# NVlabs/latentfusion

Measured on AMD Instinct MI355X. Metric: pose-optim iters/sec (reconstruct+render+backward), 16 views, 128^3 voxels, higher is better.
Workload: dtype f32

## Files before the change

### latentfusion_amd/csrc/resample.hip

```cpp
#include "resample_map.h"

namespace {

typedef unsigned u32x4_t __attribute__((ext_vector_type(4)));

struct Tap {
  int x0, y0, z0, x1, y1, z1;
  float tx, ty, tz;
  float mx, my, mz;
};

__device__ __forceinline__ float lattice01(int i, int size, float step) {
  return (i < size / 2) ? step * (float)i : 1.f - step * (float)(size - 1 - i);
}


template <int KIND>
__device__ __forceinline__ void eval_grid(const float* __restrict__ cf, int x, int y, int z,
                                          int W, int H, int D, Steps st, float& gx, float& gy, float& gz,
                                          float& a, float& b, float& k) {
  a = lattice01(x, W, st.w);
  b = lattice01(y, H, st.h);
  k = lattice01(z, D, st.d);
  if (KIND == LF_MAP_O2C) {
    const float ak = a * k, bk = b * k;
    gx = cf[0] + cf[3] * a + cf[6] * b + cf[9] * k + cf[12] * ak + cf[15] * bk;
    gy = cf[1] + cf[4] * a + cf[7] * b + cf[10] * k + cf[13] * ak + cf[16] * bk;
    gz = cf[2] + cf[5] * a + cf[8] * b + cf[11] * k + cf[14] * ak + cf[17] * bk;
  } else {
    const float lx = 2.f * a - 1.f, ly = 2.f * b - 1.f, lz = 2.f * k - 1.f;
    const float n0 = cf[0] * lx + cf[1] * ly + cf[2] * lz + cf[3];
    const float n1 = cf[4] * lx + cf[5] * ly + cf[6] * lz + cf[7];
    const float n2 = cf[8] * lx + cf[9] * ly + cf[10] * lz + cf[11];
    const float dn = cf[12] * lx + cf[13] * ly + cf[14] * lz + cf[15];
    gx = n0 / dn;
    gy = n1 / dn;
    gz = n2;
  }
}

__device__ __forceinline__ void unnormalize_clip(float g, int size, float& pos, float& mult) {
  float p = ((g + 1.f) * (float)size - 1.f) * 0.5f;
  const float hi = (float)(size - 1);
  mult = (p > 0.f && p < hi) ? 0.5f * (float)size : 0.f;
  p = fminf(fmaxf(p, 0.f), hi);
  pos = p;
}

__device__ __forceinline__ Tap make_tap(float gx, float gy, float gz, int W, int H, int D) {
  Tap t;
  float px, py, pz;
  unnormalize_clip(gx, W, px, t.mx);
  unnormalize_clip(gy, H, py, t.my);
  unnormalize_clip(gz, D, pz, t.mz);
  if (!(px == px)) px = 0.f;
  if (!(py == py)) py = 0.f;
  if (!(pz == pz)) pz = 0.f;
  const float fx = floorf(px), fy = floorf(py), fz = floorf(pz);
  t.tx = px - fx; t.ty = py - fy; t.tz = pz - fz;
  t.x0 = (int)fx; t.y0 = (int)fy; t.z0 = (int)fz;
  t.x1 = min(t.x0 + 1, W - 1); t.y1 = min(t.y0 + 1, H - 1); t.z1 = min(t.z0 + 1, D - 1);
  return t;
}

__device__ __forceinline__ unsigned xcd_contiguous(unsigned b, unsigned nb) {
  return (nb % 8 == 0) ? (b % 8) * (nb / 8) + b / 8 : b;
}

static int bwd_vox_per_block(long nvox, int N) {
  long v = nvox * N / 2048;
  int p = 64;
  while (p < 4096 && p * 2 <= v) p <<= 1;
  return p;
}
struct BwdTile { int lx, ly, lz, ntx, nty, ntz; };
static BwdTile bwd_tile(int vpb, int D, int H, int W) {
  int lg = 0;
  while ((1 << lg) < vpb) ++lg;
  BwdTile t;
  t.lx = (lg + 2) / 3; t.ly = (lg + 1) / 3; t.lz = lg / 3;
  t.ntx = (W + (1 << t.lx) - 1) >> t.lx; t.nty = (H + (1 << t.ly) - 1) >> t.ly; t.ntz = (D + (1 << t.lz) - 1) >> t.lz;
  return t;
}

__global__ void __launch_bounds__(256) resample_bwd_coef_reduce(const float* __restrict__ partial,
                                                                int nblk, float* __restrict__ gcoef) {
  const int n = blockIdx.x;
  __shared__ double red[256];
  const int comp = threadIdx.x % 18;
  const int grp = threadIdx.x / 18;
  double s = 0.0;
  if (grp < 14)
    for (int b = grp; b < nblk; b += 14) s += (double)partial[((long)n * nblk + b) * 18 + comp];
  red[threadIdx.x] = (grp < 14) ? s : 0.0;
  __syncthreads();
  if (threadIdx.x < 18) {
    double tot = 0.0;
    for (int g = 0; g < 14; ++g) tot += red[g * 18 + threadIdx.x];
    gcoef[(long)n * 18 + threadIdx.x] = (float)tot;
  }
}

template <int KIND>
__global__ void __launch_bounds__(256) resample_bwd_vol_kernel(
    const float* __restrict__ gout, const float* __restrict__ coef, float* __restrict__ gvol,
    long gvol_bstride, int N, int D, int H, int W, int C, Steps st) {
  const long per_sample = (long)D * H * W * C;
  const int n = blockIdx.y;
  const float* cf = coef + (long)n * LF_MAP_COEFS;
  for (long idx = (long)blockIdx.x * blockDim.x + threadIdx.x; idx < per_sample;
       idx += (long)gridDim.x * blockDim.x) {
    const int c = (int)(idx % C);
    long v = idx / C;
    const int x = (int)(v % W); v /= W;
    const int y = (int)(v % H);
    const int z = (int)(v / H);
    float gx, gy, gz, a, b, k;
    eval_grid<KIND>(cf, x, y, z, W, H, D, st, gx, gy, gz, a, b, k);
    const Tap t = make_tap(gx, gy, gz, W, H, D);
    const float go = gout[(long)n * per_sample + idx];
    float* base = gvol + (long)n * gvol_bstride + c;
    const long sW = C, sH = (long)W * C, sD = (long)H * W * C;
    const float wx1 = t.tx, wx0 = 1.f - t.tx, wy1 = t.ty, wy0 = 1.f - t.ty, wz1 = t.tz, wz0 = 1.f - t.tz;
    atomicAdd(base + t.z0 * sD + t.y0 * sH + t.x0 * sW, go * (wx0 * wy0 * wz0));
    atomicAdd(base + t.z0 * sD + t.y0 * sH + t.x1 * sW, go * (wx1 * wy0 * wz0));
    atomicAdd(base + t.z0 * sD + t.y1 * sH + t.x0 * sW, go * (wx0 * wy1 * wz0));
    atomicAdd(base + t.z0 * sD + t.y1 * sH + t.x1 * sW, go * (wx1 * wy1 * wz0));
    atomicAdd(base + t.z1 * sD + t.y0 * sH + t.x0 * sW, go * (wx0 * wy0 * wz1));
    atomicAdd(base + t.z1 * sD + t.y0 * sH + t.x1 * sW, go * (wx1 * wy0 * wz1));
    atomicAdd(base + t.z1 * sD + t.y1 * sH + t.x0 * sW, go * (wx0 * wy1 * wz1));
    atomicAdd(base + t.z1 * sD + t.y1 * sH + t.x1 * sW, go * (wx1 * wy1 * wz1));
  }
}

typedef unsigned u32;

struct Tap32 {
  u32 o000, o001, o010, o011, o100, o101, o110, o111;
  float tx, ty, tz, mx, my, mz;
};

__device__ __forceinline__ void axis_tap(float g, int size, u32 stride, u32& o0, u32& d1, float& t, float& m) {
  float p;
  unnormalize_clip(g, size, p, m);
  if (!(p == p)) p = 0.f;
  const float f = floorf(p);
  t = p - f;
  const int i0 = (int)f;
  o0 = (u32)i0 * stride;
  d1 = (i0 + 1 <= size - 1) ? stride : 0u;
}

__device__ __forceinline__ Tap32 make_tap32(float gx, float gy, float gz, int W, int H, int D, u32 rec_bytes) {
  Tap32 t;
  u32 x0, dx, y0, dy, z0, dz;
  axis_tap(gx, W, rec_bytes, x0, dx, t.tx, t.mx);
  axis_tap(gy, H, rec_bytes * (u32)W, y0, dy, t.ty, t.my);
  axis_tap(gz, D, rec_bytes * (u32)W * (u32)H, z0, dz, t.tz, t.mz);
  const u32 b00 = z0 + y0, b01 = b00 + dy, b10 = b00 + dz, b11 = b01 + dz;
  t.o000 = b00 + x0; t.o001 = t.o000 + dx;
  t.o010 = b01 + x0; t.o011 = t.o010 + dx;
  t.o100 = b10 + x0; t.o101 = t.o100 + dx;
  t.o110 = b11 + x0; t.o111 = t.o110 + dx;
  return t;
}

__device__ __forceinline__ f32x4 ldrec(__amdgpu_buffer_rsrc_t rs, u32 off) {
  return __builtin_bit_cast(f32x4, __builtin_amdgcn_raw_buffer_load_b128(rs, (int)off, 0, 0));
}

typedef unsigned u32x2_t __attribute__((ext_vector_type(2)));
template <bool B16>
__device__ __forceinline__ f32x4 ldrec_t(__amdgpu_buffer_rsrc_t rs, u32 off) {
  if constexpr (B16)
    return __builtin_convertvector(__builtin_bit_cast(bf16x4r, __builtin_amdgcn_raw_buffer_load_b64(rs, (int)off, 0, 0)), f32x4);
  else
    return __builtin_bit_cast(f32x4, __builtin_amdgcn_raw_buffer_load_b128(rs, (int)off, 0, 0));
}

__device__ __forceinline__ float quad_sum4(float v) {
  const float a = v + __int_as_float(__builtin_amdgcn_update_dpp(0, __float_as_int(v), 0xB1, 0xF, 0xF, true));
  return a + __int_as_float(__builtin_amdgcn_update_dpp(0, __float_as_int(a), 0x4E, 0xF, 0xF, true));
}

__device__ __forceinline__ long vol_offset(int n, long vol_bstride, const int* __restrict__ vol_idx, int vol_n) {
  const int v = vol_idx[n];
  return (long)(v < 0 ? 0 : (v >= vol_n ? vol_n - 1 : v)) * vol_bstride;
}

#define GATHER_KERNEL(stem) stem##_kernel
// ... 78 lines not shown
#endif

int g_bwd_coef_variant = 10;
int g_resample_variant = 3;

}

struct FwdPlan {
  bool vec;
  int lpt, tlx, tly, tlz, nbz;
  dim3 grid;
  Steps st;
};
static int fwd_plan(const float* vol, const float* out, int N, int D, int H, int W, int C, FwdPlan& p) {
  if ((long)D * H * W >= 0x7fffffffL) return LF_EINVAL;
  p.vec = (C % 4 == 0) && lf_aligned16(vol) && lf_aligned16(out);
  const int lpv = p.vec ? C / 4 : C;
  p.lpt = lpv < 256 ? lpv : 256;
  int lg = 0;
  while ((2 << lg) * p.lpt <= 256) ++lg;
  if (lg >= 6) { p.tlx = (lg + 2) / 3; p.tly = (lg + 1) / 3; p.tlz = lg / 3; }
  else         { p.tlx = lg < 2 ? lg : 2; p.tly = lg - p.tlx < 2 ? lg - p.tlx : 2; p.tlz = lg - p.tlx - p.tly; }
  p.nbz = (D + (1 << p.tlz) - 1) >> p.tlz;
  const int nby = (H + (1 << p.tly) - 1) >> p.tly;
  if ((long)p.nbz * N > 65535 || nby > 65535) return LF_EINVAL;
  p.grid = dim3((unsigned)((W + (1 << p.tlx) - 1) >> p.tlx), (unsigned)nby, (unsigned)(p.nbz * N));
  p.st = make_steps(D, H, W);
  return 0;
}

extern "C" int lf_resample3d_fwd(const float* vol, int vol_n, const float* coef, int kind, float* out,
                                 int N, int D, int H, int W, int C, void* stream) {
  lf_clear_error();
  if (N <= 0 || D <= 0 || H <= 0 || W <= 0 || C <= 0) return LF_EINVAL;
  if (vol_n != 1 && vol_n != N) return LF_EINVAL;
  if (kind != LF_MAP_O2C && kind != LF_MAP_C2O) return LF_EINVAL;
  const long bstride = vol_n == 1 ? 0 : (long)D * H * W * C;
  FwdPlan p;
  if (int e = fwd_plan(vol, out, N, D, H, W, C, p)) return e;
  hipStream_t s = (hipStream_t)stream;
  if (g_resample_variant == 4 && p.vec && C == 16 && (long)D * H * W * 64 < 0xffffffffL && W <= 65535) {
    const int ntx = (W + LT_X - 1) / LT_X, nty = (H + LT_Y - 1) / LT_Y, ntz = (D + LT_Z - 1) / LT_Z;
    const long nwg = (long)ntx * nty * ntz * N;
    if (nwg > 0x7fffffffL) return LF_EINVAL;
    LAUNCH_BY_KIND(resample_fwd_staged_kernel, dim3((unsigned)nwg), vol, bstride, coef, out, D, H, W, ntx, nty, ntz, p.st);
    return lf_launch_status();
  }
  if (g_resample_variant == 5 && p.vec && C == 16 && (long)D * H * W * 64 < 0xffffffffL) {
    const int nbz4 = (D + 3) >> 2, nbx16 = (W + 15) >> 4, nby4 = (H + 3) >> 2;
    if ((long)nbz4 * N > 65535 || nby4 > 65535) return LF_EINVAL;
    dim3 g5((unsigned)nbx16, (unsigned)nby4, (unsigned)(nbz4 * N));
    LAUNCH_BY_KIND(resample_fwd_c16_dedup_kernel, g5, vol, bstride, coef, out, D, H, W, nbx16, nby4, nbz4, p.st);
    return lf_launch_status();
  }
  if (g_resample_variant >= 3 && p.vec && C == 16 && (long)D * H * W * 64 < 0xffffffffL) {
    LAUNCH_BY_KIND(resample_fwd_c16_kernel, p.grid, vol, bstride, coef, out, D, H, W, p.nbz, p.st);
  } else if (g_resample_variant >= 2 && p.vec && (long)D * H * W * C * 4 < 0xffffffffL) {
    LAUNCH_BY_KIND(resample_fwd_lean_kernel, p.grid, vol, bstride, coef, out, D, H, W, C, p.lpt, p.tlx, p.tly, p.tlz, p.nbz, p.st);
  } else {
#define LAUNCH(K, V) hipLaunchKernelGGL((resample_fwd_kernel<K, V>), p.grid, dim3(256), 0, s, vol, bstride, coef, out, N, D, H, W, C, p.lpt, p.tlx, p.tly, p.tlz, p.nbz, p.st)
    if (kind == LF_MAP_O2C) { if (p.vec) LAUNCH(LF_MAP_O2C, 4); else LAUNCH(LF_MAP_O2C, 1); }
    else                    { if (p.vec) LAUNCH(LF_MAP_C2O, 4); else LAUNCH(LF_MAP_C2O, 1); }
#undef LAUNCH
  }
  return lf_launch_status();
}

static long staged_bwd_blocks(int D, int H, int W) {
  const long nt = (long)((W + LT_X - 1) / LT_X) * ((H + LT_Y - 1) / LT_Y) * ((D + LT_Z - 1) / LT_Z);
  return (nt + STAGED_TPW - 1) / STAGED_TPW;
}

static size_t bwd_coef_scratch_bytes(int N, int part_n, int D, int H, int W) {
  const long nvox = (long)D * H * W;
  const int vpb = bwd_vox_per_block(nvox, part_n);
  const BwdTile bt = bwd_tile(vpb, D, H, W);
  const long nblk = (long)bt.ntx * bt.nty * bt.ntz;
  const long nblk_staged = staged_bwd_blocks(D, H, W);
  return (size_t)N * (nblk > nblk_staged ? nblk : nblk_staged) * 18 * sizeof(float);
}

extern "C" size_t lf_resample3d_bwd_coef_scratch_bytes(int N, int D, int H, int W) {
  return bwd_coef_scratch_bytes(N, N, D, H, W);
}

extern "C" size_t lf_resample3d_bwd_coef_part_scratch_bytes(int N, int part_n, int D, int H, int W) {
  if (N <= 0 || part_n <= 0) return 0;
  return bwd_coef_scratch_bytes(N, part_n, D, H, W);
}

struct BwdCoefPlan {
  long nvox;
  int vpb, nblk, lpv;
  BwdTile bt;
  bool vec;
  dim3 grid;
  Steps st;
};
static int bwd_coef_plan(const float* gout, const float* vol, size_t scratch_bytes, int N, int part_n, int D, int H, int W, int C,
                         BwdCoefPlan& p) {
  if (scratch_bytes < bwd_coef_scratch_bytes(N, part_n, D, H, W)) return LF_ENOSPC;
  if ((long)D * H * W >= 0x7fffffffL) return LF_EINVAL;
  p.nvox = (long)D * H * W;
  p.vpb = bwd_vox_per_block(p.nvox, part_n);
  p.bt = bwd_tile(p.vpb, D, H, W);
  const long nblk_l = (long)p.bt.ntx * p.bt.nty * p.bt.ntz;
  if (nblk_l * N > 0x7fffffffL) return LF_EINVAL;
  p.nblk = (int)nblk_l;
  p.grid = dim3((unsigned)(nblk_l * N));
  p.vec = (C % 4 == 0) && lf_aligned16(gout) && lf_aligned16(vol);
  const int groups = p.vec ? C / 4 : C;
  p.lpv = 1;
  while (p.lpv < groups) p.lpv <<= 1;
  if (p.lpv > 64) return LF_EINVAL;
  p.st = make_steps(D, H, W);
  return 0;
}

static int bwd_coef_finish(const float* partial, int nblk, float* gcoef, int N, hipStream_t s) {
  if (int e = lf_launch_status()) return e;
  hipLaunchKernelGGL(resample_bwd_coef_reduce, dim3(N), dim3(256), 0, s, partial, nblk, gcoef);
  return lf_launch_status();
}

static int bwd_coef_launch(const float* gout, const float* vol, int vol_n, const float* coef,
                           float* gcoef, void* scratch, size_t scratch_bytes,
                           int N, int part_n, int D, int H, int W, int C, void* stream) {
  if (N <= 0 || D <= 0 || H <= 0 || W <= 0 || C <= 0) return LF_EINVAL;
  if (vol_n != 1 && vol_n != N) return LF_EINVAL;
  BwdCoefPlan p;
  if (int e = bwd_coef_plan(gout, vol, scratch_bytes, N, part_n, D, H, W, C, p)) return e;
  const long bstride = vol_n == 1 ? 0 : p.nvox * C;
  hipStream_t s = (hipStream_t)stream;
  float* partial = (float*)scratch;
  if (g_resample_variant == 4 && p.vec && C == 16 && p.nvox * 64 < 0xffffffffL && W <= 65535) {
    const int ntx = (W + LT_X - 1) / LT_X, nty = (H + LT_Y - 1) / LT_Y, ntz = (D + LT_Z - 1) / LT_Z;
    const long nb = staged_bwd_blocks(D, H, W);
    if (nb * N > 0x7fffffffL) return LF_EINVAL;
    hipLaunchKernelGGL((resample_bwd_coef_staged_kernel<STAGED_TPW>), dim3((unsigned)(nb * N)), dim3(256), 0, s, gout, vol, bstride, coef,
                       partial, (int)nb, D, H, W, ntx, nty, ntz, p.st);
    return bwd_coef_finish(partial, (int)nb, gcoef, N, s);
  }
  if (g_resample_variant >= 2 && p.vec && C == 16 && p.vpb >= 64 && p.nvox * 64 < 0xffffffffL) {
    const int v = g_bwd_coef_variant;
    const bool big = p.vpb >= 256;
#define LAUNCH(...) hipLaunchKernelGGL((__VA_ARGS__), p.grid, dim3(256), 0, s, gout, vol, bstride, coef, partial, p.nblk, p.vpb, p.bt, D, H, W, p.st)
    if (v == 1)              LAUNCH(resample_bwd_coef_c16_kernel<1, 1>);
    else if (v == 2)         LAUNCH(resample_bwd_coef_c16_kernel<1, 2>);
    else if (v == 3)         LAUNCH(resample_bwd_coef_c16_kernel<4, 2>);
    else if (v == 6 && big)  LAUNCH(resample_bwd_coef_c16_dedup_kernel<2, 1>);
    else if (v == 7 && big)  LAUNCH(resample_bwd_coef_c16_dedup_kernel<1, 1>);
    else if (v == 8 && big)  LAUNCH(resample_bwd_coef_c16_dedup_kernel<2, 4>);
    else if (v == 9 && big)  LAUNCH(resample_bwd_coef_c16_dedup_kernel<1, 5>);
    else if (v == 10 && big) LAUNCH(resample_bwd_coef_c16_dedup_kernel<2, 1, true>);
    else if (v == 11 && big) LAUNCH(resample_bwd_coef_c16_dedup_kernel<1, 1, true>);
    else if (v == 4)         LAUNCH(resample_bwd_coef_c16_kernel<6, 1>);
    else                     LAUNCH(resample_bwd_coef_c16_kernel<8, 1>);
#undef LAUNCH
  } else if (p.vec) {
    hipLaunchKernelGGL((resample_bwd_coef_kernel<4>), p.grid, dim3(256), 0, s, gout, vol, bstride, coef, partial, p.nblk, p.vpb, p.bt, N, D, H, W, C, p.lpv, p.st);
  } else {
    hipLaunchKernelGGL((resample_bwd_coef_kernel<1>), p.grid, dim3(256), 0, s, gout, vol, bstride, coef, partial, p.nblk, p.vpb, p.bt, N, D, H, W, C, p.lpv, p.st);
  }
  return bwd_coef_finish(partial, p.nblk, gcoef, N, s);
}

extern "C" int lf_resample3d_bwd_coef(const float* gout, const float* vol, int vol_n, const float* coef,
                                      float* gcoef, void* scratch, size_t scratch_bytes,
                                      int N, int D, int H, int W, int C, void* stream) {
  lf_clear_error();
  return bwd_coef_launch(gout, vol, vol_n, coef, gcoef, scratch, scratch_bytes, N, N, D, H, W, C, stream);
}

extern "C" int lf_resample3d_bwd_coef_part(const float* gout, const float* vol, int vol_n, const float* coef,
                                           float* gcoef, void* scratch, size_t scratch_bytes,
                                           int N, int D, int H, int W, int C, int part_n, void* stream) {
  lf_clear_error();
  if (!gout || !vol || !coef || !gcoef || !scratch) return LF_EINVAL;
  if (part_n <= 0 || N <= 0) return LF_EINVAL;
  return bwd_coef_launch(gout, vol, vol_n, coef, gcoef, scratch, scratch_bytes, N, part_n, D, H, W, C, stream);
}

extern "C" int lf_resample3d_fwd_indexed(const float* vol, int vol_n, const int* vol_idx, const float* coef, int kind, float* out,
                                         int N, int D, int H, int W, int C, void* stream) {
  lf_clear_error();
  if (!vol || !vol_idx || !coef || !out) return LF_EINVAL;
  if (N <= 0 || D <= 0 || H <= 0 || W <= 0 || C <= 0 || vol_n < 1) return LF_EINVAL;
  if (kind != LF_MAP_O2C && kind != LF_MAP_C2O) return LF_EINVAL;
  if (((uintptr_t)vol_idx & 3) != 0) return LF_EALIGN;
  const long bstride = (long)D * H * W * C;
  FwdPlan p;
  if (int e = fwd_plan(vol, out, N, D, H, W, C, p)) return e;
  hipStream_t s = (hipStream_t)stream;
  if (g_resample_variant >= 3 && p.vec && C == 16 && (long)D * H * W * 64 < 0xffffffffL) {
    LAUNCH_BY_KIND(resample_fwd_c16_indexed_kernel, p.grid, vol, bstride, vol_idx, vol_n, coef, out, D, H, W, p.nbz, p.st);
  } else if (g_resample_variant >= 2 && p.vec && (long)D * H * W * C * 4 < 0xffffffffL) {
    LAUNCH_BY_KIND(resample_fwd_lean_indexed_kernel, p.grid, vol, bstride, vol_idx, vol_n, coef, out, D, H, W, C, p.lpt, p.tlx, p.tly, p.tlz, p.nbz, p.st);
  } else {
#define LAUNCH(K, V) hipLaunchKernelGGL((resample_fwd_indexed_kernel<K, V>), p.grid, dim3(256), 0, s, vol, bstride, vol_idx, vol_n, coef, out, N, D, H, W, C, p.lpt, p.tlx, p.tly, p.tlz, p.nbz, p.st)
    if (kind == LF_MAP_O2C) { if (p.vec) LAUNCH(LF_MAP_O2C, 4); else LAUNCH(LF_MAP_O2C, 1); }
    else                    { if (p.vec) LAUNCH(LF_MAP_C2O, 4); else LAUNCH(LF_MAP_C2O, 1); }
#undef LAUNCH
  }
  return lf_launch_status();
}

extern "C" size_t lf_resample3d_bwd_coef_indexed_scratch_bytes(int N, int part_n, int D, int H, int W) {
  if (N <= 0 || part_n <= 0) return 0;
  return bwd_coef_scratch_bytes(N, part_n, D, H, W);
}

extern "C" int lf_resample3d_bwd_coef_indexed(const float* gout, const float* vol, int vol_n, const int* vol_idx, const float* coef,
                                              float* gcoef, void* scratch, size_t scratch_bytes,
                                              int N, int D, int H, int W, int C, int part_n, void* stream) {
  lf_clear_error();
  if (!gout || !vol || !vol_idx || !coef || !gcoef || !scratch) return LF_EINVAL;
  if (part_n <= 0 || N <= 0 || vol_n < 1) return LF_EINVAL;
  if (D <= 0 || H <= 0 || W <= 0 || C <= 0) return LF_EINVAL;
  if (((uintptr_t)vol_idx & 3) != 0) return LF_EALIGN;
  BwdCoefPlan p;
  if (int e = bwd_coef_plan(gout, vol, scratch_bytes, N, part_n, D, H, W, C, p)) return e;
  const long bstride = p.nvox * C;
  hipStream_t s = (hipStream_t)stream;
  float* partial = (float*)scratch;
  if (g_resample_variant >= 2 && p.vec && C == 16 && p.vpb >= 64 && p.nvox * 64 < 0xffffffffL) {
    if (p.vpb >= 256)
      hipLaunchKernelGGL((resample_bwd_coef_c16_dedup_indexed_kernel<2, 1, true>), p.grid, dim3(256), 0, s, gout, vol, bstride, vol_idx, vol_n, coef, partial, p.nblk, p.vpb, p.bt, D, H, W, p.st);
    else
      hipLaunchKernelGGL((resample_bwd_coef_c16_indexed_kernel<8, 1>), p.grid, dim3(256), 0, s, gout, vol, bstride, vol_idx, vol_n, coef, partial, p.nblk, p.vpb, p.bt, D, H, W, p.st);
  } else if (p.vec) {
    hipLaunchKernelGGL((resample_bwd_coef_indexed_kernel<4>), p.grid, dim3(256), 0, s, gout, vol, bstride, vol_idx, vol_n, coef, partial, p.nblk, p.vpb, p.bt, N, D, H, W, C, p.lpv, p.st);
  } else {
    hipLaunchKernelGGL((resample_bwd_coef_indexed_kernel<1>), p.grid, dim3(256), 0, s, gout, vol, bstride, vol_idx, vol_n, coef, partial, p.nblk, p.vpb, p.bt, N, D, H, W, C, p.lpv, p.st);
  }
  return bwd_coef_finish(partial, p.nblk, gcoef, N, s);
}

extern "C" int lf_resample3d_bwd_vol(const float* gout, const float* coef, int kind, float* gvol, int vol_n,
                                     int N, int D, int H, int W, int C, void* stream) {
  lf_clear_error();
  if (N <= 0 || D <= 0 || H <= 0 || W <= 0 || C <= 0) return LF_EINVAL;
  if (vol_n != 1 && vol_n != N) return LF_EINVAL;
  const long bstride = vol_n == 1 ? 0 : (long)D * H * W * C;
  const long items = (long)D * H * W * C;
  dim3 grid((unsigned)min((items + 255) / 256, (long)65535 * 16), N), block(256);
  hipStream_t s = (hipStream_t)stream;
  if (kind == LF_MAP_O2C)
    hipLaunchKernelGGL((resample_bwd_vol_kernel<LF_MAP_O2C>), grid, block, 0, s, gout, coef, gvol, bstride, N, D, H, W, C, make_steps(D, H, W));
  else if (kind == LF_MAP_C2O)
    hipLaunchKernelGGL((resample_bwd_vol_kernel<LF_MAP_C2O>), grid, block, 0, s, gout, coef, gvol, bstride, N, D, H, W, C, make_steps(D, H, W));
  else
    return LF_EINVAL;
  return lf_launch_status();
}

#ifdef STAGE_TS
extern "C" int lf_debug_stage_ts(void* dst) {
  return (int)hipMemcpyFromSymbol(dst, HIP_SYMBOL(g_stage_ts), sizeof(unsigned long long) * 256 * 16, 0, hipMemcpyDeviceToHost);
}
#endif

extern "C" int lf_set_tuning(int key, int value) {
  if (key == 1) {
    const int prev = g_resample_variant;
    if (value >= 1 && value <= 5) g_resample_variant = value;
    return prev;
  }
  if (key == 4) return lf_internal_splat_set_variant(value);
  if (key == 6) return lf_internal_splat_set_chunk_cap(value);
  if (key == 3) return lf_internal_fused_set_cfg(value);
  if (key == 7) return lf_internal_wino_set_pack(value);
  if (key == 8) return lf_internal_wino_set_forms(value);
  if (key == 5) return lf_internal_ring_bf16_set_wgs(value);
  if (key == 2) {
    const int prev = g_bwd_coef_variant;
    if (value >= 1 && value <= 11) g_bwd_coef_variant = value;
    return prev;
  }
  return LF_EINVAL;
}

extern "C" int lf_resample3d_fwd_io(const void* vol, int vol_n, const float* coef, int kind, void* out,
                                    int N, int D, int H, int W, int io, void* stream) {
  lf_clear_error();
  if (N <= 0 || D <= 0 || H <= 0 || W <= 0 || io < 0 || io > 3) return LF_EINVAL;
  if ((vol_n != 1 && vol_n != N) || (kind != LF_MAP_O2C && kind != LF_MAP_C2O)) return LF_EINVAL;
  if (!lf_aligned16(vol) || !lf_aligned16(out)) return LF_EALIGN;
  if ((long)D * H * W * 64 >= 0xffffffffL) return LF_EINVAL;
  const long bstride = vol_n == 1 ? 0 : (long)D * H * W * 16;
  const int nbz4 = (D + 3) >> 2;
  if ((long)nbz4 * N > 65535 || ((H + 3) >> 2) > 65535) return LF_EINVAL;
  dim3 g4((unsigned)((W + 3) >> 2), (unsigned)((H + 3) >> 2), (unsigned)(nbz4 * N)), block(256);
  const Steps st = make_steps(D, H, W);
  typedef void (*kern_t)(const float*, long, const float*, float*, int, int, int, int, Steps);
  static const kern_t kerns[2][4] = {
      {resample_fwd_c16_kernel<LF_MAP_O2C, 0>, resample_fwd_c16_kernel<LF_MAP_O2C, 1>, resample_fwd_c16_kernel<LF_MAP_O2C, 2>, resample_fwd_c16_kernel<LF_MAP_O2C, 3>},
      {resample_fwd_c16_kernel<LF_MAP_C2O, 0>, resample_fwd_c16_kernel<LF_MAP_C2O, 1>, resample_fwd_c16_kernel<LF_MAP_C2O, 2>, resample_fwd_c16_kernel<LF_MAP_C2O, 3>}};
  hipLaunchKernelGGL(kerns[kind == LF_MAP_O2C ? 0 : 1][io], g4, block, 0, (hipStream_t)stream, (const float*)vol, bstride, coef, (float*)out, D, H, W, nbz4, st);
  return lf_launch_status();
}
```

### latentfusion_amd/csrc/resample_gather.inc

```

template <int KIND, int VEC>
__global__ void __launch_bounds__(256) GATHER_KERNEL(resample_fwd)(
    const float* __restrict__ vol, long vol_bstride, GATHER_TABLE_PARAMS const float* __restrict__ coef,
    float* __restrict__ out, int N, int D, int H, int W, int C, int lpt, int lx, int ly, int lz, int nbz, Steps st) {
  const int lpv = C / VEC;
  const int n = blockIdx.z / nbz, bz = blockIdx.z - n * nbz;
  const int slot = threadIdx.x / lpt, q0 = threadIdx.x - slot * lpt;
  if (slot >= (1 << (lx + ly + lz))) return;
  const int x = (blockIdx.x << lx) + (slot & ((1 << lx) - 1));
  const int y = (blockIdx.y << ly) + ((slot >> lx) & ((1 << ly) - 1));
  const int z = (bz << lz) + (slot >> (lx + ly));
  if (x >= W || y >= H || z >= D) return;
  const float* cf = coef + (long)n * LF_MAP_COEFS;
  float gx, gy, gz, a, b, k;
  eval_grid<KIND>(cf, x, y, z, W, H, D, st, gx, gy, gz, a, b, k);
  const Tap t = make_tap(gx, gy, gz, W, H, D);
  const float wx1 = t.tx, wx0 = 1.f - t.tx, wy1 = t.ty, wy0 = 1.f - t.ty, wz1 = t.tz, wz0 = 1.f - t.tz;
  const float w000 = wx0 * wy0 * wz0, w001 = wx1 * wy0 * wz0, w010 = wx0 * wy1 * wz0, w011 = wx1 * wy1 * wz0;
  const float w100 = wx0 * wy0 * wz1, w101 = wx1 * wy0 * wz1, w110 = wx0 * wy1 * wz1, w111 = wx1 * wy1 * wz1;
  const int r00 = (t.z0 * H + t.y0) * W, r01 = (t.z0 * H + t.y1) * W;
  const int r10 = (t.z1 * H + t.y0) * W, r11 = (t.z1 * H + t.y1) * W;
  const float* base = vol + GATHER_VOL_OFFSET;
  float* orow = out + ((long)n * D * H * W + ((long)z * H + y) * W + x) * C;
  for (int q = q0; q < lpv; q += lpt) {
// ... 101 lines not shown

template <int KIND>
__global__ void __launch_bounds__(256) GATHER_KERNEL(resample_fwd_lean)(
    const float* __restrict__ vol, long vol_bstride, GATHER_TABLE_PARAMS const float* __restrict__ coef,
    float* __restrict__ out, int D, int H, int W, int C, int lpt, int lx, int ly, int lz, int nbz, Steps st) {
  const int lpv = C >> 2;
  const int n = blockIdx.z / nbz, bz = blockIdx.z - n * nbz;
  const int slot = threadIdx.x / lpt, q0 = threadIdx.x - slot * lpt;
  if (slot >= (1 << (lx + ly + lz))) return;
  const int x = (blockIdx.x << lx) + (slot & ((1 << lx) - 1));
  const int y = (blockIdx.y << ly) + ((slot >> lx) & ((1 << ly) - 1));
  const int z = (bz << lz) + (slot >> (lx + ly));
  if (x >= W || y >= H || z >= D) return;
  const u32 rec = (u32)C * 4u;
  const u32 sample_bytes = (u32)D * (u32)H * (u32)W * rec;
  const __amdgpu_buffer_rsrc_t rs = __builtin_amdgcn_make_buffer_rsrc((void*)(vol + GATHER_VOL_OFFSET), 0, sample_bytes, 0x00020000);
  const __amdgpu_buffer_rsrc_t ro = __builtin_amdgcn_make_buffer_rsrc((void*)(out + (long)n * D * H * W * C), 0, sample_bytes, 0x00020000);
  const float* cf = coef + n * LF_MAP_COEFS;
  float gx, gy, gz, a, b, k;
  eval_grid<KIND>(cf, x, y, z, W, H, D, st, gx, gy, gz, a, b, k);
  const Tap32 t = make_tap32(gx, gy, gz, W, H, D, rec);
  const float wx1 = t.tx, wx0 = 1.f - t.tx, wy1 = t.ty, wy0 = 1.f - t.ty, wz1 = t.tz, wz0 = 1.f - t.tz;
  const float w000 = wx0 * wy0 * wz0, w001 = wx1 * wy0 * wz0, w010 = wx0 * wy1 * wz0, w011 = wx1 * wy1 * wz0;
  const float w100 = wx0 * wy0 * wz1, w101 = wx1 * wy0 * wz1, w110 = wx0 * wy1 * wz1, w111 = wx1 * wy1 * wz1;
  const u32 orow = (u32)((z * H + y) * W + x) * rec;
  for (int q = q0; q < lpv; q += lpt) {
    const u32 co = (u32)q * 16u;
    const f32x4 v000 = ldrec(rs, t.o000 + co), v001 = ldrec(rs, t.o001 + co), v010 = ldrec(rs, t.o010 + co), v011 = ldrec(rs, t.o011 + co);
    const f32x4 v100 = ldrec(rs, t.o100 + co), v101 = ldrec(rs, t.o101 + co), v110 = ldrec(rs, t.o110 + co), v111 = ldrec(rs, t.o111 + co);
    const f32x4 r = v000 * w000 + v001 * w001 + v010 * w010 + v011 * w011 + v100 * w100 + v101 * w101 + v110 * w110 + v111 * w111;
    __builtin_amdgcn_raw_buffer_store_b128(__builtin_bit_cast(u32x4_t, r), ro, (int)(orow + co), 0, 2);
  }
}

template <int KIND, int IO = 0>
__global__ void __launch_bounds__(256) GATHER_KERNEL(resample_fwd_c16)(
    const float* __restrict__ vol, long vol_bstride, GATHER_TABLE_PARAMS const float* __restrict__ coef,
    float* __restrict__ out, int D, int H, int W, int nbz, Steps st) {
  constexpr bool IN16 = (IO & 1) != 0, OUT16 = (IO & 2) != 0;
  constexpr u32 IREC = IN16 ? 32u : 64u, OREC = OUT16 ? 32u : 64u;
  const int n = blockIdx.z / nbz, bz = blockIdx.z - n * nbz;
  const int q = threadIdx.x & 3, vs = threadIdx.x >> 2;
  const int x = (blockIdx.x << 2) + (vs & 3), y = (blockIdx.y << 2) + ((vs >> 2) & 3), z = (bz << 2) + (vs >> 4);
  if (x >= W || y >= H || z >= D) return;
  const u32 nvox = (u32)D * (u32)H * (u32)W;
  const __amdgpu_buffer_rsrc_t rs = __builtin_amdgcn_make_buffer_rsrc((void*)((const char*)vol + GATHER_VOL_OFFSET * (IN16 ? 2 : 4)), 0, nvox * IREC, 0x00020000);
  const __amdgpu_buffer_rsrc_t ro = __builtin_amdgcn_make_buffer_rsrc((void*)((char*)out + (long)n * nvox * OREC), 0, nvox * OREC, 0x00020000);
  const float* cf = coef + n * LF_MAP_COEFS;
  float gx, gy, gz, a, b, k;
  eval_grid<KIND>(cf, x, y, z, W, H, D, st, gx, gy, gz, a, b, k);
  const Tap32 t = make_tap32(gx, gy, gz, W, H, D, IREC);
  const u32 co = (u32)q * (IREC / 4u);
  const f32x4 v000 = ldrec_t<IN16>(rs, t.o000 + co), v001 = ldrec_t<IN16>(rs, t.o001 + co), v010 = ldrec_t<IN16>(rs, t.o010 + co), v011 = ldrec_t<IN16>(rs, t.o011 + co);
  const f32x4 v100 = ldrec_t<IN16>(rs, t.o100 + co), v101 = ldrec_t<IN16>(rs, t.o101 + co), v110 = ldrec_t<IN16>(rs, t.o110 + co), v111 = ldrec_t<IN16>(rs, t.o111 + co);
  const float wx1 = t.tx, wx0 = 1.f - t.tx, wy1 = t.ty, wy0 = 1.f - t.ty, wz1 = t.tz, wz0 = 1.f - t.tz;
  const float w000 = wx0 * wy0 * wz0, w001 = wx1 * wy0 * wz0, w010 = wx0 * wy1 * wz0, w011 = wx1 * wy1 * wz0;
  const float w100 = wx0 * wy0 * wz1, w101 = wx1 * wy0 * wz1, w110 = wx0 * wy1 * wz1, w111 = wx1 * wy1 * wz1;
  f32x4 r;
#pragma unroll
  for (int e = 0; e < 4; ++e) {
    float acc = v000[e] * w000;
    asm("v_fmac_f32 %0, %1, %2" : "+v"(acc) : "v"(v001[e]), "v"(w001));
    asm("v_fmac_f32 %0, %1, %2" : "+v"(acc) : "v"(v010[e]), "v"(w010));
    asm("v_fmac_f32 %0, %1, %2" : "+v"(acc) : "v"(v011[e]), "v"(w011));
    asm("v_fmac_f32 %0, %1, %2" : "+v"(acc) : "v"(v100[e]), "v"(w100));
    asm("v_fmac_f32 %0, %1, %2" : "+v"(acc) : "v"(v101[e]), "v"(w101));
    asm("v_fmac_f32 %0, %1, %2" : "+v"(acc) : "v"(v110[e]), "v"(w110));
    asm("v_fmac_f32 %0, %1, %2" : "+v"(acc) : "v"(v111[e]), "v"(w111));
    r[e] = acc;
  }
  if constexpr (OUT16)
    __builtin_amdgcn_raw_buffer_store_b64(__builtin_bit_cast(u32x2_t, __builtin_convertvector(r, bf16x4r)), ro,
                                          (int)((u32)((z * H + y) * W + x) * 32u + (u32)q * 8u), 0, 2);
  else
    __builtin_amdgcn_raw_buffer_store_b128(__builtin_bit_cast(u32x4_t, r), ro, (int)((u32)((z * H + y) * W + x) * 64u + (u32)q * 16u), 0, 2);
}

template <int MINW, int UNR>
__global__ void __launch_bounds__(256, MINW) GATHER_KERNEL(resample_bwd_coef_c16)(
    const float* __restrict__ gout, const float* __restrict__ vol, long vol_bstride, GATHER_TABLE_PARAMS
    const float* __restrict__ coef, float* __restrict__ partial, int nblk, int vpb, BwdTile bt,
    int D, int H, int W, Steps st) {
  const unsigned fb = xcd_contiguous(blockIdx.x, gridDim.x);
  const int n = fb / nblk, blk = fb - n * nblk;
  const float* cf = coef + n * LF_MAP_COEFS;
  const u32 rec = 64u;
  const u32 sample_bytes = (u32)D * (u32)H * (u32)W * rec;
  const __amdgpu_buffer_rsrc_t rs = __builtin_amdgcn_make_buffer_rsrc((void*)(vol + GATHER_VOL_OFFSET), 0, sample_bytes, 0x00020000);
  const __amdgpu_buffer_rsrc_t rg = __builtin_amdgcn_make_buffer_rsrc((void*)(gout + (long)n * D * H * W * 16), 0, sample_bytes, 0x00020000);
  const int tx = blk % bt.ntx, ty = (blk / bt.ntx) % bt.nty, tz = blk / (bt.ntx * bt.nty);
  const int q = threadIdx.x & 3, vs = threadIdx.x >> 2;
  const int px = vs & 3, py = (vs >> 2) & 3, pz = vs >> 4;
  const int sbx = bt.lx - 2, sby = bt.ly - 2;
  float acc[6];
#pragma unroll
  for (int i = 0; i < 6; ++i) acc[i] = 0.f;
  const int nsub = vpb >> 6;
  const u32 co = (u32)q * 16u;
  for (int sub0 = 0; sub0 < nsub; sub0 += UNR) {
    Tap32 t[UNR];
    float a[UNR], b[UNR], k[UNR];
    f32x4 go[UNR], v[UNR][8];
#pragma unroll
    for (int u = 0; u < UNR; ++u) {
      const int sub = sub0 + u;
      const int x = (tx << bt.lx) + ((sub & ((1 << sbx) - 1)) << 2) + px;
      const int y = (ty << bt.ly) + (((sub >> sbx) & ((1 << sby) - 1)) << 2) + py;
      const int z = (tz << bt.lz) + ((sub >> (sbx + sby)) << 2) + pz;
      const bool live = sub < nsub && x < W && y < H && z < D;
      float gx, gy, gz;
      eval_grid<LF_MAP_O2C>(cf, live ? x : 0, live ? y : 0, live ? z : 0, W, H, D, st, gx, gy, gz, a[u], b[u], k[u]);
      t[u] = make_tap32(gx, gy, gz, W, H, D, rec);
      const u32 dead = live ? 0u : 0xffffffffu;
      go[u] = __builtin_bit_cast(f32x4, __builtin_amdgcn_raw_buffer_load_b128(
          rg, (int)(((u32)((z * H + y) * W + x) * rec + co) | dead), 0, 2));
      v[u][0] = ldrec(rs, (t[u].o000 + co) | dead); v[u][1] = ldrec(rs, (t[u].o001 + co) | dead);
      v[u][2] = ldrec(rs, (t[u].o010 + co) | dead); v[u][3] = ldrec(rs, (t[u].o011 + co) | dead);
      v[u][4] = ldrec(rs, (t[u].o100 + co) | dead); v[u][5] = ldrec(rs, (t[u].o101 + co) | dead);
      v[u][6] = ldrec(rs, (t[u].o110 + co) | dead); v[u][7] = ldrec(rs, (t[u].o111 + co) | dead);
    }
#pragma unroll
    for (int u = 0; u < UNR; ++u) {
      float p[8];
#pragma unroll
      for (int c8 = 0; c8 < 8; ++c8)
        p[c8] = quad_sum4((go[u][0] * v[u][c8][0] + go[u][1] * v[u][c8][1]) + (go[u][2] * v[u][c8][2] + go[u][3] * v[u][c8][3]));
      const float wx1 = t[u].tx, wx0 = 1.f - wx1, wy1 = t[u].ty, wy0 = 1.f - wy1, wz1 = t[u].tz, wz0 = 1.f - wz1;
      const float dxv = (p[1] - p[0]) * (wy0 * wz0) + (p[3] - p[2]) * (wy1 * wz0) + (p[5] - p[4]) * (wy0 * wz1) + (p[7] - p[6]) * (wy1 * wz1);
      const float dyv = (p[2] - p[0]) * (wx0 * wz0) + (p[3] - p[1]) * (wx1 * wz0) + (p[6] - p[4]) * (wx0 * wz1) + (p[7] - p[5]) * (wx1 * wz1);
      const float dzv = (p[4] - p[0]) * (wx0 * wy0) + (p[5] - p[1]) * (wx1 * wy0) + (p[6] - p[2]) * (wx0 * wy1) + (p[7] - p[3]) * (wx1 * wy1);
      const float hx = dxv * t[u].mx, hy = dyv * t[u].my, hz = dzv * t[u].mz;
      const float B0 = q == 0 ? 1.f : (q == 1 ? b[u] : (q == 2 ? a[u] * k[u] : 0.f));
      const float B1 = q == 0 ? a[u] : (q == 1 ? k[u] : (q == 2 ? b[u] * k[u] : 0.f));
      acc[0] += hx * B0; acc[1] += hy * B0; acc[2] += hz * B0;
      acc[3] += hx * B1; acc[4] += hy * B1; acc[5] += hz * B1;
    }
  }
  __shared__ double red[4][18];
  const int wave = threadIdx.x >> 6, lane = threadIdx.x & 63;
#pragma unroll
  for (int i = 0; i < 6; ++i) {
    double s = (double)acc[i];
#pragma unroll
    for (int o = 32; o >= 4; o >>= 1) s += __shfl_xor(s, o, 64);
    if (lane < 3) red[wave][(2 * lane + i / 3) * 3 + (i % 3)] = s;
  }
  __syncthreads();
  if (threadIdx.x < 18) {
    const double s = (red[0][threadIdx.x] + red[1][threadIdx.x]) + (red[2][threadIdx.x] + red[3][threadIdx.x]);
    partial[((long)n * nblk + blk) * 18 + threadIdx.x] = (float)s;
  }
}

template <int PIF, int MINW, bool GOPF = false>
__global__ void __launch_bounds__(256, MINW) GATHER_KERNEL(resample_bwd_coef_c16_dedup)(
    const float* __restrict__ gout, const float* __restrict__ vol, long vol_bstride, GATHER_TABLE_PARAMS
    const float* __restrict__ coef, float* __restrict__ partial, int nblk, int vpb, BwdTile bt,
    int D, int H, int W, Steps st) {
  __shared__ u32x4_t tapbuf[4][64];
  __shared__ float pbuf[4][64 * 8];
  __shared__ double red[4][18];
  const unsigned fb = xcd_contiguous(blockIdx.x, gridDim.x);
  const int n = fb / nblk, blk = fb - n * nblk;
  const float* cf = coef + n * LF_MAP_COEFS;
  const u32 rec = 64u;
  const u32 sample_bytes = (u32)D * (u32)H * (u32)W * rec;
  const __amdgpu_buffer_rsrc_t rs = __builtin_amdgcn_make_buffer_rsrc((void*)(vol + GATHER_VOL_OFFSET), 0, sample_bytes, 0x00020000);
  const __amdgpu_buffer_rsrc_t rg = __builtin_amdgcn_make_buffer_rsrc((void*)(gout + (long)n * D * H * W * 16), 0, sample_bytes, 0x00020000);
  const int tx = blk % bt.ntx, ty = (blk / bt.ntx) % bt.nty, tz = blk / (bt.ntx * bt.nty);
  const int lane = threadIdx.x & 63, wave = threadIdx.x >> 6;
  const int px = lane & 3, py = (lane >> 2) & 3, pz = lane >> 4;
  const int q = lane & 3, vq = lane >> 2;
  const int sbx = bt.lx - 2, sby = bt.ly - 2;
  const int nsub = vpb >> 6;
  const u32 co = (u32)q * 16u;
  float acc[18];
#pragma unroll
  for (int i = 0; i < 18; ++i) acc[i] = 0.f;
  u32x4_t* tb = tapbuf[wave];
  float* pb = pbuf[wave];
  f32x4 gnext[4];
  auto load_go = [&](int sub_, f32x4 (&dst)[4]) {
    const int bx0 = (tx << bt.lx) + ((sub_ & ((1 << sbx) - 1)) << 2);
    const int by0 = (ty << bt.ly) + (((sub_ >> sbx) & ((1 << sby) - 1)) << 2);
    const int bz0 = (tz << bt.lz) + ((sub_ >> (sbx + sby)) << 2);
#pragma unroll
    for (int i = 0; i < 4; ++i) {
      const int vi = 16 * i + vq;
      const int vx = bx0 + (vi & 3), vy = by0 + ((vi >> 2) & 3), vz = bz0 + (vi >> 4);
      const u32 dead = (sub_ < nsub && vx < W && vy < H && vz < D) ? 0u : 0xffffffffu;
      dst[i] = __builtin_bit_cast(f32x4, __builtin_amdgcn_raw_buffer_load_b128(
          rg, (int)(((u32)((vz * H + vy) * W + vx) * rec + co) | dead), 0, 2));
    }
  };
  if (GOPF) load_go(wave, gnext);
  for (int sub = wave; sub < nsub; sub += 4) {
    const int x0 = (tx << bt.lx) + ((sub & ((1 << sbx) - 1)) << 2);
    const int y0 = (ty << bt.ly) + (((sub >> sbx) & ((1 << sby) - 1)) << 2);
    const int z0 = (tz << bt.lz) + ((sub >> (sbx + sby)) << 2);
    f32x4 gcur[4];
    if (GOPF) {
#pragma unroll
      for (int i = 0; i < 4; ++i) gcur[i] = gnext[i];
      load_go(sub + 4, gnext);
    }
    const int x = x0 + px, y = y0 + py, z = z0 + pz;
    const bool live = x < W && y < H && z < D;
    float gx, gy, gz, a, b, k;
    eval_grid<LF_MAP_O2C>(cf, live ? x : 0, live ? y : 0, live ? z : 0, W, H, D, st, gx, gy, gz, a, b, k);
    u32 ox, dx, oy, dy, oz, dz;
    float tx_, ty_, tz_, mx, my, mz;
    axis_tap(gx, W, rec, ox, dx, tx_, mx);
    axis_tap(gy, H, rec * (u32)W, oy, dy, ty_, my);
    axis_tap(gz, D, rec * (u32)W * (u32)H, oz, dz, tz_, mz);
    u32x4_t tr;
    tr[0] = live ? (oz + oy + ox) : 0xffffffffu;
    tr[1] = live ? dx : 0u; tr[2] = live ? dy : 0u; tr[3] = live ? dz : 0u;
    tb[lane] = tr;
    asm volatile("s_waitcnt lgkmcnt(0)" ::: "memory");
#pragma unroll 1
    for (int i0 = 0; i0 < 4; i0 += (GOPF ? 4 : PIF)) {
      if (GOPF) {
#pragma unroll
        for (int j0 = 0; j0 < 4; j0 += PIF) {
          f32x4 v[PIF][8];
#pragma unroll
          for (int u = 0; u < PIF; ++u) {
            const u32x4_t t = tb[16 * (j0 + u) + vq];
            const u32 dead = t[0] == 0xffffffffu ? 0xffffffffu : 0u;
            const u32 b00 = (t[0] + co) | dead, b01 = b00 + t[2], b10 = b00 + t[3], b11 = b01 + t[3];
            v[u][0] = ldrec(rs, b00); v[u][1] = ldrec(rs, b00 + t[1]);
            v[u][2] = ldrec(rs, b01); v[u][3] = ldrec(rs, b01 + t[1]);
            v[u][4] = ldrec(rs, b10); v[u][5] = ldrec(rs, b10 + t[1]);
            v[u][6] = ldrec(rs, b11); v[u][7] = ldrec(rs, b11 + t[1]);
          }
#pragma unroll
          for (int u = 0; u < PIF; ++u) {
            const f32x4 go = gcur[j0 + u];
            float p[8];
#pragma unroll
            for (int c8 = 0; c8 < 8; ++c8)
              p[c8] = quad_sum4((go[0] * v[u][c8][0] + go[1] * v[u][c8][1]) + (go[2] * v[u][c8][2] + go[3] * v[u][c8][3]));
            const float e0 = q == 0 ? p[0] : (q == 1 ? p[2] : (q == 2 ? p[4] : p[6]));
            const float e1 = q == 0 ? p[1] : (q == 1 ? p[3] : (q == 2 ? p[5] : p[7]));
            *(float2*)(pb + (16 * (j0 + u) + vq) * 8 + 2 * q) = make_float2(e0, e1);
          }
          __builtin_amdgcn_sched_barrier(0);
        }
        continue;
      }
      f32x4 go[PIF], v[PIF][8];
#pragma unroll
      for (int u = 0; u < PIF; ++u) {
        const int vi = 16 * (i0 + u) + vq;
        const u32x4_t t = tb[vi];
        const int vx = x0 + (vi & 3), vy = y0 + ((vi >> 2) & 3), vz = z0 + (vi >> 4);
        const u32 dead = t[0] == 0xffffffffu ? 0xffffffffu : 0u;
        go[u] = __builtin_bit_cast(f32x4, __builtin_amdgcn_raw_buffer_load_b128(
            rg, (int)(((u32)((vz * H + vy) * W + vx) * rec + co) | dead), 0, 2));
        const u32 b00 = (t[0] + co) | dead, b01 = b00 + t[2], b10 = b00 + t[3], b11 = b01 + t[3];
        v[u][0] = ldrec(rs, b00); v[u][1] = ldrec(rs, b00 + t[1]);
        v[u][2] = ldrec(rs, b01); v[u][3] = ldrec(rs, b01 + t[1]);
        v[u][4] = ldrec(rs, b10); v[u][5] = ldrec(rs, b10 + t[1]);
        v[u][6] = ldrec(rs, b11); v[u][7] = ldrec(rs, b11 + t[1]);
      }
#pragma unroll
      for (int u = 0; u < PIF; ++u) {
        float p[8];
#pragma unroll
        for (int c8 = 0; c8 < 8; ++c8)
          p[c8] = quad_sum4((go[u][0] * v[u][c8][0] + go[u][1] * v[u][c8][1]) + (go[u][2] * v[u][c8][2] + go[u][3] * v[u][c8][3]));
        const float e0 = q == 0 ? p[0] : (q == 1 ? p[2] : (q == 2 ? p[4] : p[6]));
        const float e1 = q == 0 ? p[1] : (q == 1 ? p[3] : (q == 2 ? p[5] : p[7]));
        *(float2*)(pb + (16 * (i0 + u) + vq) * 8 + 2 * q) = make_float2(e0, e1);
      }
    }
    asm volatile("s_waitcnt lgkmcnt(0)" ::: "memory");
    {
      const f32x4 pa = *(const f32x4*)(pb + lane * 8), pc = *(const f32x4*)(pb + lane * 8 + 4);
      const float wx1 = tx_, wx0 = 1.f - wx1, wy1 = ty_, wy0 = 1.f - wy1, wz1 = tz_, wz0 = 1.f - wz1;
      const float dxv = (pa[1] - pa[0]) * (wy0 * wz0) + (pa[3] - pa[2]) * (wy1 * wz0) + (pc[1] - pc[0]) * (wy0 * wz1) + (pc[3] - pc[2]) * (wy1 * wz1);
      const float dyv = (pa[2] - pa[0]) * (wx0 * wz0) + (pa[3] - pa[1]) * (wx1 * wz0) + (pc[2] - pc[0]) * (wx0 * wz1) + (pc[3] - pc[1]) * (wx1 * wz1);
      const float dzv = (pc[0] - pa[0]) * (wx0 * wy0) + (pc[1] - pa[1]) * (wx1 * wy0) + (pc[2] - pa[2]) * (wx0 * wy1) + (pc[3] - pa[3]) * (wx1 * wy1);
      const float hx = live ? dxv * mx : 0.f, hy = live ? dyv * my : 0.f, hz = live ? dzv * mz : 0.f;
      const float ak = a * k, bk = b * k;
      acc[0] += hx;       acc[1] += hy;       acc[2] += hz;
      acc[3] += hx * a;   acc[4] += hy * a;   acc[5] += hz * a;
      acc[6] += hx * b;   acc[7] += hy * b;   acc[8] += hz * b;
      acc[9] += hx * k;   acc[10] += hy * k;  acc[11] += hz * k;
      acc[12] += hx * ak; acc[13] += hy * ak; acc[14] += hz * ak;
      acc[15] += hx * bk; acc[16] += hy * bk; acc[17] += hz * bk;
    }
    asm volatile("" ::: "memory");
  }
#pragma unroll
  for (int i = 0; i < 18; ++i) {
    double s = (double)acc[i];
#pragma unroll
    for (int o = 32; o > 0; o >>= 1) s += __shfl_xor(s, o, 64);
    if (lane == 0) red[wave][i] = s;
  }
  __syncthreads();
  if (threadIdx.x < 18) {
    const double s = (red[0][threadIdx.x] + red[1][threadIdx.x]) + (red[2][threadIdx.x] + red[3][threadIdx.x]);
    partial[((long)n * nblk + blk) * 18 + threadIdx.x] = (float)s;
  }
}
```

Measured before the change: 193.0.

## Add LDS-staged grad-out prefetch variant for dedup coef-backward kernel

Adds a GOPF==2 mode to the dedup coefficient-gradient kernel. It prefetches the next subtile's grad-output directly into LDS with buffer_load_lds, and parks per-lane tap weights and lattice coords in shared memory to relieve registers. The mode also pins the FMA ordering of the O2C grid evaluation so results stay consistent. It is selectable as tuning variant 12 for both plain and indexed launchers, at the cost of extra LDS use and explicit vmcnt waits.

After: 190.9. 0.989x the previous value.

```diff
diff --git a/latentfusion_amd/csrc/resample.hip b/latentfusion_amd/csrc/resample.hip
--- a/latentfusion_amd/csrc/resample.hip
+++ b/latentfusion_amd/csrc/resample.hip
@@ -36,6 +36,20 @@
     gx = n0 / dn;
     gy = n1 / dn;
     gz = n2;
+  }
+}
+
+__device__ __forceinline__ void eval_grid_o2c_pinned(const float* __restrict__ cf, int x, int y, int z, int W, int H, int D, Steps st,
+                                                     float& gx, float& gy, float& gz, float& a, float& b, float& k) {
+  a = lattice01(x, W, st.w);
+  b = lattice01(y, H, st.h);
+  k = lattice01(z, D, st.d);
+  {
+#pragma clang fp contract(off)
+    const float ak = a * k, bk = b * k;
+    gx = __builtin_fmaf(cf[15], bk, __builtin_fmaf(cf[12], ak, __builtin_fmaf(cf[9], k, __builtin_fmaf(cf[6], b, __builtin_fmaf(cf[3], a, cf[0])))));
+    gy = __builtin_fmaf(cf[16], bk, __builtin_fmaf(cf[13], ak, __builtin_fmaf(cf[10], k, __builtin_fmaf(cf[7], b, __builtin_fmaf(cf[4], a, cf[1])))));
+    gz = (((__builtin_fmaf(cf[5], a, cf[2]) + cf[8] * b) + cf[11] * k) + cf[14] * ak) + cf[17] * bk;
   }
 }
 
@@ -420,8 +434,9 @@
     else if (v == 7 && big)  LAUNCH(resample_bwd_coef_c16_dedup_kernel<1, 1>);
     else if (v == 8 && big)  LAUNCH(resample_bwd_coef_c16_dedup_kernel<2, 4>);
     else if (v == 9 && big)  LAUNCH(resample_bwd_coef_c16_dedup_kernel<1, 5>);
-    else if (v == 10 && big) LAUNCH(resample_bwd_coef_c16_dedup_kernel<2, 1, true>);
-    else if (v == 11 && big) LAUNCH(resample_bwd_coef_c16_dedup_kernel<1, 1, true>);
+    else if (v == 10 && big) LAUNCH(resample_bwd_coef_c16_dedup_kernel<2, 1, 1>);
+    else if (v == 11 && big) LAUNCH(resample_bwd_coef_c16_dedup_kernel<1, 1, 1>);
+    else if (v == 12 && big) LAUNCH(resample_bwd_coef_c16_dedup_kernel<2, 4, 2>);
     else if (v == 4)         LAUNCH(resample_bwd_coef_c16_kernel<6, 1>);
     else                     LAUNCH(resample_bwd_coef_c16_kernel<8, 1>);
 #undef LAUNCH
@@ -492,8 +507,10 @@
   hipStream_t s = (hipStream_t)stream;
   float* partial = (float*)scratch;
   if (g_resample_variant >= 2 && p.vec && C == 16 && p.vpb >= 64 && p.nvox * 64 < 0xffffffffL) {
-    if (p.vpb >= 256)
-      hipLaunchKernelGGL((resample_bwd_coef_c16_dedup_indexed_kernel<2, 1, true>), p.grid, dim3(256), 0, s, gout, vol, bstride, vol_idx, vol_n, coef, partial, p.nblk, p.vpb, p.bt, D, H, W, p.st);
+    if (p.vpb >= 256 && g_bwd_coef_variant == 12)
+      hipLaunchKernelGGL((resample_bwd_coef_c16_dedup_indexed_kernel<2, 4, 2>), p.grid, dim3(256), 0, s, gout, vol, bstride, vol_idx, vol_n, coef, partial, p.nblk, p.vpb, p.bt, D, H, W, p.st);
+    else if (p.vpb >= 256)
+      hipLaunchKernelGGL((resample_bwd_coef_c16_dedup_indexed_kernel<2, 1, 1>), p.grid, dim3(256), 0, s, gout, vol, bstride, vol_idx, vol_n, coef, partial, p.nblk, p.vpb, p.bt, D, H, W, p.st);
     else
       hipLaunchKernelGGL((resample_bwd_coef_c16_indexed_kernel<8, 1>), p.grid, dim3(256), 0, s, gout, vol, bstride, vol_idx, vol_n, coef, partial, p.nblk, p.vpb, p.bt, D, H, W, p.st);
   } else if (p.vec) {
@@ -542,7 +559,7 @@
   if (key == 5) return lf_internal_ring_bf16_set_wgs(value);
   if (key == 2) {
     const int prev = g_bwd_coef_variant;
-    if (value >= 1 && value <= 11) g_bwd_coef_variant = value;
+    if (value >= 1 && value <= 12) g_bwd_coef_variant = value;
     return prev;
   }
   return LF_EINVAL;
diff --git a/latentfusion_amd/csrc/resample_gather.inc b/latentfusion_amd/csrc/resample_gather.inc
--- a/latentfusion_amd/csrc/resample_gather.inc
+++ b/latentfusion_amd/csrc/resample_gather.inc
@@ -277,7 +277,7 @@
   }
 }
 
-template <int PIF, int MINW, bool GOPF = false>
+template <int PIF, int MINW, int GOPF = 0>
 __global__ void __launch_bounds__(256, MINW) GATHER_KERNEL(resample_bwd_coef_c16_dedup)(
     const float* __restrict__ gout, const float* __restrict__ vol, long vol_bstride, GATHER_TABLE_PARAMS
     const float* __restrict__ coef, float* __restrict__ partial, int nblk, int vpb, BwdTile bt,
@@ -318,13 +318,35 @@
           rg, (int)(((u32)((vz * H + vy) * W + vx) * rec + co) | dead), 0, 2));
     }
   };
-  if (GOPF) load_go(wave, gnext);
+  f32x4* gs = nullptr;
+  f32x4* cs = nullptr;
+  float* ks = nullptr;
+  if constexpr (GOPF == 2) {
+    __shared__ f32x4 gobuf[4][256];
+    __shared__ f32x4 cbuf[4][128];
+    __shared__ float kbuf[4][64];
+    gs = gobuf[wave]; cs = cbuf[wave]; ks = kbuf[wave];
+  }
+  auto stage_go = [&](int sub_) {
+    const int bx0 = (tx << bt.lx) + ((sub_ & ((1 << sbx) - 1)) << 2);
+    const int by0 = (ty << bt.ly) + (((sub_ >> sbx) & ((1 << sby) - 1)) << 2);
+    const int bz0 = (tz << bt.lz) + ((sub_ >> (sbx + sby)) << 2);
+#pragma unroll
+    for (int i = 0; i < 4; ++i) {
+      const int vx = bx0 + (vq & 3), vy = by0 + (vq >> 2), vz = bz0 + i;
+      const u32 dead = (sub_ < nsub && vx < W && vy < H && vz < D) ? 0u : 0xffffffffu;
+      __builtin_amdgcn_raw_ptr_buffer_load_lds(rg, (__attribute__((address_space(3))) void*)(gs + 64 * i), 16,
+                                               (int)(((u32)((vz * H + vy) * W + vx) * rec + co) | dead), 0, 0, 2);
+    }
+  };
+  if (GOPF == 1) load_go(wave, gnext);
+  if constexpr (GOPF == 2) stage_go(wave);
   for (int sub = wave; sub < nsub; sub += 4) {
     const int x0 = (tx << bt.lx) + ((sub & ((1 << sbx) - 1)) << 2);
     const int y0 = (ty << bt.ly) + (((sub >> sbx) & ((1 << sby) - 1)) << 2);
     const int z0 = (tz << bt.lz) + ((sub >> (sbx + sby)) << 2);
     f32x4 gcur[4];
-    if (GOPF) {
+    if (GOPF == 1) {
 #pragma unroll
       for (int i = 0; i < 4; ++i) gcur[i] = gnext[i];
       load_go(sub + 4, gnext);
@@ -332,7 +354,10 @@
     const int x = x0 + px, y = y0 + py, z = z0 + pz;
     const bool live = x < W && y < H && z < D;
     float gx, gy, gz, a, b, k;
-    eval_grid<LF_MAP_O2C>(cf, live ? x : 0, live ? y : 0, live ? z : 0, W, H, D, st, gx, gy, gz, a, b, k);
+    if constexpr (GOPF == 2)
+      eval_grid_o2c_pinned(cf, live ? x : 0, live ? y : 0, live ? z : 0, W, H, D, st, gx, gy, gz, a, b, k);
+    else
+      eval_grid<LF_MAP_O2C>(cf, live ? x : 0, live ? y : 0, live ? z : 0, W, H, D, st, gx, gy, gz, a, b, k);
     u32 ox, dx, oy, dy, oz, dz;
     float tx_, ty_, tz_, mx, my, mz;
     axis_tap(gx, W, rec, ox, dx, tx_, mx);
@@ -342,6 +367,11 @@
     tr[0] = live ? (oz + oy + ox) : 0xffffffffu;
     tr[1] = live ? dx : 0u; tr[2] = live ? dy : 0u; tr[3] = live ? dz : 0u;
     tb[lane] = tr;
+    if constexpr (GOPF == 2) {
+      cs[lane] = (f32x4){tx_, ty_, tz_, a};
+      cs[64 + lane] = (f32x4){mx, my, mz, b};
+      ks[lane] = k;
+    }
     asm volatile("s_waitcnt lgkmcnt(0)" ::: "memory");
 #pragma unroll 1
     for (int i0 = 0; i0 < 4; i0 += (GOPF ? 4 : PIF)) {
@@ -359,9 +389,14 @@
             v[u][4] = ldrec(rs, b10); v[u][5] = ldrec(rs, b10 + t[1]);
             v[u][6] = ldrec(rs, b11); v[u][7] = ldrec(rs, b11 + t[1]);
           }
+          if constexpr (GOPF == 2) {
+            __builtin_amdgcn_sched_barrier(0);
+            if (j0 == 0) asm volatile("s_waitcnt vmcnt(%0)" ::"n"(8 * PIF) : "memory");
+          }
 #pragma unroll
           for (int u = 0; u < PIF; ++u) {
-            const f32x4 go = gcur[j0 + u];
+            f32x4 go;
+            if constexpr (GOPF == 2) go = gs[64 * (j0 + u) + lane]; else go = gcur[j0 + u];
             float p[8];
 #pragma unroll
             for (int c8 = 0; c8 < 8; ++c8)
@@ -401,7 +436,14 @@
       }
     }
     asm volatile("s_waitcnt lgkmcnt(0)" ::: "memory");
+    if constexpr (GOPF == 2) stage_go(sub + 4);
     {
+      if constexpr (GOPF == 2) {
+        const f32x4 c0 = cs[lane], c1 = cs[64 + lane];
+        tx_ = c0[0]; ty_ = c0[1]; tz_ = c0[2]; a = c0[3];
+        mx = c1[0]; my = c1[1]; mz = c1[2]; b = c1[3];
+        k = ks[lane];
+      }
       const f32x4 pa = *(const f32x4*)(pb + lane * 8), pc = *(const f32x4*)(pb + lane * 8 + 4);
       const float wx1 = tx_, wx0 = 1.f - wx1, wy1 = ty_, wy0 = 1.f - wy1, wz1 = tz_, wz0 = 1.f - wz1;
       const float dxv = (pa[1] - pa[0]) * (wy0 * wz0) + (pa[3] - pa[2]) * (wy1 * wz0) + (pc[1] - pc[0]) * (wy0 * wz1) + (pc[3] - pc[2]) * (wy1 * wz1);
@@ -418,6 +460,7 @@
     }
     asm volatile("" ::: "memory");
   }
+  if constexpr (GOPF == 2) asm volatile("s_waitcnt vmcnt(0)" ::: "memory");
 #pragma unroll
   for (int i = 0; i < 18; ++i) {
     double s = (double)acc[i];
```
